# vainglorygame/analyzer

Hardware: AMD Instinct MI355X
Metric: matches/sec rated (whole node), 3v3 TrueSkill, 1M-player roster (higher is better)
Workload: dtype fp32; 1 GPU; global_batch=10000000, seq_len=6, players=1000000, matches_per_gpu=10000000, team_size=3, parallelism=dp1, mode=exact, bench_config=2, skew=1, force_merge=False

## Files before the change

analyzer_amd/csrc/common.h:

```cpp
#pragma once

#include <stdint.h>

#include <type_traits>

#ifndef ANA_DIAG_BUILD
#define ANA_DIAG_BUILD 0
#endif

#if defined(__HIPCC__)
#include <hip/hip_runtime.h>
#define ANA_HD __host__ __device__ __forceinline__
#else
#define ANA_HD inline
#endif

namespace ana {

constexpr int kTracks = 7;
constexpr int kGranules = 8;
constexpr int kRowFloats = 32;
constexpr int kBaseFloats = 16;
constexpr int kLinkWords = 1;
constexpr uint32_t kNoMatch = 0x0fffffffu;
constexpr uint32_t kMatchMask = 0x0fffffffu;
constexpr uint32_t kLinkHasPred = 1u << 30;
constexpr uint32_t kNone = 0xffffffffu;
constexpr int kSlotBits = 28;
constexpr int64_t kMaxSlots = 1ll << kSlotBits;
constexpr int kModes = 6;
constexpr int kModeUnsupported = 255;
constexpr int kVstTiers = 31;
constexpr int kMaxTeamSize = 5;

enum Status : uint8_t {
  kRated = 0,
  kAfk = 1,
  kInvalidRosters = 2,
  kUnsupportedMode = 3,
  kErrSeed = 4,
  kErrSigma = 5,
  kErrEmptyRoster = 6,
  kErrNumeric = 7,
  kErrBadRecord = 8,
  kNotProcessed = 255,
};

struct RateParams {
  float beta2;
  float tau2;
  float unknown_sigma;
  int32_t num_players;
  int64_t num_matches;
  int32_t record_first_prior;
  int32_t epoch;
  const int32_t* epoch_ptr;
  const float* vst;
  int32_t idle_spins;
  int32_t tight_groups;
  int32_t local_handoff;
  int32_t diag;
  uint64_t* progress;
  uint64_t progress_value;
  int64_t progress_at;
  int32_t chunk_len;
  int32_t ctrl_ready;
};

struct RateOut {
  float* quality;
  uint8_t* status;
  float* s_mu;
  float* s_sig;
  float* delta;
  float* m_mu;
  float* m_sig;
  int64_t row;
  int64_t qrow;
  int64_t srow;
};

ANA_HD int meta_mode(uint32_t m0) { return (int)(m0 & 0xffu); }
ANA_HD int meta_n0(uint32_t m0) { return (int)((m0 >> 8) & 0xffu); }
ANA_HD int meta_n1(uint32_t m0) { return (int)((m0 >> 16) & 0xffu); }
ANA_HD int meta_nrosters(uint32_t m0) { return (int)((m0 >> 24) & 0xffu); }
ANA_HD bool meta_winner0(uint32_t m1) { return (m1 & 1u) != 0; }
ANA_HD bool meta_winner1(uint32_t m1) { return (m1 & 2u) != 0; }
ANA_HD bool meta_afk(uint32_t m1) { return (m1 & 4u) != 0; }
ANA_HD uint32_t pack_meta0(int mode, int n0, int n1, int nrosters) {
  return (uint32_t)(mode & 0xff) | ((uint32_t)(n0 & 0xff) << 8) |
         ((uint32_t)(n1 & 0xff) << 16) | ((uint32_t)(nrosters & 0xff) << 24);
}
ANA_HD uint32_t pack_meta1(bool w0, bool w1, uint32_t afk_mask) {
  return (w0 ? 1u : 0u) | (w1 ? 2u : 0u) | (afk_mask ? 4u : 0u) | ((afk_mask & 0xffffffu) << 8);
}

template <int K>
ANA_HD uint8_t early_status(const int32_t* r, int64_t P) {
  constexpr int S = 2 * K;
  const uint32_t m0 = (uint32_t)r[S], m1 = (uint32_t)r[S + 1];
  const int n0 = meta_n0(m0), n1 = meta_n1(m0);
  bool bad = n0 > K || n1 > K;
#pragma unroll
  for (int j = 0; j < S; ++j) {
    const int pos = j < K ? j : j - K;
    if (pos < (j < K ? n0 : n1) && (r[j] < 0 || (int64_t)r[j] >= P)) bad = true;
  }
  if (meta_mode(m0) >= kModes) return kUnsupportedMode;
  if (bad) return kErrBadRecord;
  if (meta_nrosters(m0) != 2) return kInvalidRosters;
  if (meta_afk(m1)) return kAfk;
  return kRated;
}

ANA_HD uint8_t early_status_k(const int32_t* r, int S, int64_t P) {
  switch (S / 2) {
    case 1: return early_status<1>(r, P);
    case 2: return early_status<2>(r, P);
    case 3: return early_status<3>(r, P);
    case 4: return early_status<4>(r, P);
    case 5: return early_status<5>(r, P);
    default: return kErrBadRecord;
  }
}

template <class F>
inline bool with_team_size(int K, F&& f) {
  switch (K) {
    case 1: f(std::integral_constant<int, 1>{}); return true;
    case 2: f(std::integral_constant<int, 2>{}); return true;
    case 3: f(std::integral_constant<int, 3>{}); return true;
    case 4: f(std::integral_constant<int, 4>{}); return true;
    case 5: f(std::integral_constant<int, 5>{}); return true;
    default: return false;
  }
}
static_assert(kMaxTeamSize == 5, "with_team_size and early_status_k list the team sizes");

inline bool window_ok(int K, int64_t W, int64_t M, int64_t P) {
  return K >= 1 && K <= kMaxTeamSize && W >= 5 * 2 * K + 2 && M >= 0 && P >= 0 && P <= 0x7fffffffll;
}
inline bool window_slots_ok(int K, int64_t W, int64_t M, int64_t P) {
  return window_ok(K, W, M, P) && M * 2 * K <= kMaxSlots;
}
inline bool sorted_slots_ok(int K, int64_t n, int64_t P) {
  return K >= 1 && K <= kMaxTeamSize && n >= 0 && n <= kMaxSlots && n % (2 * K) == 0 && P >= 0 && P <= 0x7fffffffll;
}

ANA_HD uint64_t mix64(uint64_t z) {
  z += 0x9e3779b97f4a7c15ull;
  z = (z ^ (z >> 30)) * 0xbf58476d1ce4e5b9ull;
  z = (z ^ (z >> 27)) * 0x94d049bb133111ebull;
  return z ^ (z >> 31);
}
ANA_HD uint64_t rng_u64(uint64_t seed, uint64_t index, uint32_t field) {
  return mix64(mix64(seed ^ (0xd1b54a32d192ed03ull * (uint64_t)(field + 1))) + index);
}
ANA_HD float rng_unit(uint64_t seed, uint64_t index, uint32_t field) {
  return (float)(rng_u64(seed, index, field) >> 40) * (1.0f / 16777216.0f);
}

}
```

analyzer_amd/csrc/radix_sort.hip:

```cpp
#include <hip/hip_runtime.h>

#include <cstdlib>

#include "common.h"
#include "kernels.h"
#include "record_dev.h"

namespace ana {

namespace {

constexpr int kThreads = 512;
constexpr int kWaves = kThreads / 64;
constexpr int kItems = 16;
constexpr int kTile = kThreads * kItems;
constexpr int kRadixBits = 8;
constexpr int kRadix = 1 << kRadixBits;
static_assert(kRadix <= kThreads, "one digit per thread");

__device__ __forceinline__ int64_t xcd_tile(int64_t tiles) {
  const int64_t i = blockIdx.x, q = tiles >> 3, r = tiles & 7, x = i & 7;
  return x * q + (x < r ? x : r) + (i >> 3);
}

template <bool NT>
__device__ __forceinline__ uint32_t ld32(const uint32_t* p) {
  if constexpr (NT) return __builtin_nontemporal_load(p);
  else return *p;
}

__device__ __forceinline__ uint32_t block_exclusive_scan(uint32_t x, uint32_t* wsum,
                                                         uint32_t* total) {
  const int lane = threadIdx.x & 63, wv = threadIdx.x >> 6;
  uint32_t inc = x;
#pragma unroll
  for (int off = 1; off < 64; off <<= 1) {
    const uint32_t y = __shfl_up(inc, off);
    if (lane >= off) inc += y;
  }
  if (lane == 63) wsum[wv] = inc;
  __syncthreads();
  uint32_t before = 0, all = 0;
#pragma unroll
  for (int w = 0; w < kWaves; ++w) {
    if (w < wv) before += wsum[w];
    all += wsum[w];
  }
  if (total) *total = all;
  __syncthreads();
  return before + inc - x;
}

template <int KS>
__device__ __forceinline__ void decode_tile_keys(const int32_t* __restrict__ rec, uint32_t kend,
                                                 int64_t base, int64_t n, uint32_t* lk, uint32_t knone) {
  constexpr int S = 2 * KS, R = S + 2;
  const uint32_t lo = (uint32_t)base;
  const uint32_t hi = (uint32_t)(base + kTile < n ? base + kTile : n);
  const uint32_t m_lo = lo / S, m_hi = (hi + S - 1) / S;
  for (uint32_t m = m_lo + threadIdx.x; m < m_hi; m += kThreads) {
    uint32_t key[S];
    sched_slot_keys<KS>(rec + (int64_t)m * R, (int64_t)kend, knone, key);
#pragma unroll
    for (int j = 0; j < S; ++j) {
      const uint32_t slot = m * S + j;
      if (slot >= lo && slot < hi) lk[slot - lo] = key[j];
    }
  }
}

struct SchedInit {
  int32_t* deps = nullptr;
  uint32_t* ctrl = nullptr;
  int nz = 0;
  int32_t* epoch_bump = nullptr;
};

template <int KS, bool NT = false>
__global__ void __launch_bounds__(kThreads)
radix_upsweep(const uint32_t* __restrict__ keys, const int32_t* __restrict__ rec, uint32_t kend,
              int64_t n, int shift, uint32_t* __restrict__ counts, int64_t tiles, SchedInit init = {},
              uint32_t knone = 0u) {
  __shared__ uint32_t hist[kWaves][kRadix];
  __shared__ uint32_t lkeys[KS > 0 ? kTile : 1];
  const int tid = threadIdx.x, wv = tid >> 6;
  for (int i = tid; i < kWaves * kRadix; i += kThreads) (&hist[0][0])[i] = 0u;
  const int64_t tile = xcd_tile(tiles);
  const int64_t base = tile * kTile;
  if constexpr (KS > 0) {
    if (init.deps) {
      constexpr int S = 2 * KS;
      const int64_t hi = base + kTile < n ? base + kTile : n;
      for (int64_t m = (base + S - 1) / S + tid; m < (hi + S - 1) / S; m += kThreads) init.deps[m] = 0;
    }
    if (blockIdx.x == 0) {
      if (tid < init.nz) init.ctrl[tid] = 0u;
      if (tid == 0 && init.epoch_bump) init.epoch_bump[0] += 1;
    }
  }
  if constexpr (KS > 0) decode_tile_keys<KS>(rec, kend, base, n, lkeys, knone ? knone : kend);
  __syncthreads();
#pragma unroll
  for (int k = 0; k < kItems; ++k) {
    const int64_t idx = base + k * kThreads + tid;
    if (idx < n) {
      const uint32_t key = KS > 0 ? lkeys[k * kThreads + tid] : ld32<NT>(keys + idx);
      atomicAdd(&hist[wv][(key >> shift) & (kRadix - 1)], 1u);
    }
  }
  __syncthreads();
#pragma unroll
  for (int d = tid; d < kRadix; d += kThreads) {
    uint32_t c = 0;
#pragma unroll
    for (int w = 0; w < kWaves; ++w) c += hist[w][d];
    counts[(int64_t)d * tiles + tile] = c;
  }
}

__global__ void __launch_bounds__(kThreads)
radix_rowscan(uint32_t* __restrict__ counts, int64_t tiles, uint32_t* __restrict__ totals) {
  __shared__ uint32_t wsum[kWaves];
  constexpr int kPer = 4;
  uint32_t* row = counts + (int64_t)blockIdx.x * tiles;
  uint32_t carry = 0;
  for (int64_t start = 0; start < tiles; start += kThreads * kPer) {
    uint32_t v[kPer], s = 0;
#pragma unroll
    for (int q = 0; q < kPer; ++q) {
      const int64_t t = start + (int64_t)threadIdx.x * kPer + q;
      v[q] = t < tiles ? row[t] : 0u;
      s += v[q];
    }
    uint32_t all;
    uint32_t ex = carry + block_exclusive_scan(s, wsum, &all);
#pragma unroll
    for (int q = 0; q < kPer; ++q) {
      const int64_t t = start + (int64_t)threadIdx.x * kPer + q;
      if (t < tiles) row[t] = ex;
      ex += v[q];
    }
    carry += all;
  }
  if (threadIdx.x == 0) totals[blockIdx.x] = carry;
}

struct RunEnds {
  uint32_t kf, vf, kl, vl;
};
constexpr uint32_t kRunEmpty = 0xffffffffu;

template <int KS, bool LINK, bool NT = false>
__global__ void __launch_bounds__(kThreads)
radix_downsweep(const uint32_t* __restrict__ kin, const uint32_t* __restrict__ vin,
                const int32_t* __restrict__ rec, uint32_t kend,
                uint32_t* __restrict__ kout, uint32_t* __restrict__ vout, int64_t n, int shift,
                const uint32_t* __restrict__ counts, const uint32_t* __restrict__ totals,
                int64_t tiles, int slots_per_match, uint32_t* __restrict__ link,
                uint32_t vlo = 0u, uint32_t vhi = 0xffffffffu, int bounds = 1,
                RunEnds* __restrict__ bnd = nullptr, int nd = 0, uint32_t knone = 0u) {
  __shared__ uint32_t skey[kTile];
  __shared__ uint32_t sval[kTile];
  __shared__ uint32_t wcnt[kWaves][kRadix];
  __shared__ uint32_t tstart[kRadix];
  __shared__ uint32_t gstart[kRadix];
  __shared__ uint32_t wsum[kWaves];
  const int tid = threadIdx.x, lane = tid & 63, wv = tid >> 6;
  const int64_t tile = xcd_tile(tiles);
  const int64_t base = tile * kTile;
  for (int i = tid; i < kWaves * kRadix; i += kThreads) (&wcnt[0][0])[i] = 0u;
  const bool local_ends = LINK && bnd != nullptr;
  if (!local_ends) {
    const uint32_t below = block_exclusive_scan(tid < kRadix ? totals[tid] : 0u, wsum, nullptr);
    if (tid < kRadix) gstart[tid] = below + counts[(int64_t)tid * tiles + tile];
  }
  if constexpr (KS > 0)
    decode_tile_keys<KS>(rec, kend, base, n, sval, knone ? knone : kend);
  __syncthreads();

  const uint64_t lt_mask = (1ull << lane) - 1ull;
  uint32_t key[kItems], val[kItems], rank[kItems];
#pragma unroll
  for (int it = 0; it < kItems; ++it) {
    const int64_t idx = base + (int64_t)(wv * kItems + it) * 64 + lane;
    const bool valid = idx < n;
    if constexpr (KS > 0) key[it] = valid ? sval[(wv * kItems + it) * 64 + lane] : 0xffffffffu;
    else key[it] = valid ? ld32<NT>(kin + idx) : 0xffffffffu;
    if constexpr (KS == 0) val[it] = valid ? ld32<NT>(vin + idx) : 0u;
    else val[it] = (uint32_t)idx;
  }
#pragma unroll
  for (int it = 0; it < kItems; ++it) {
    const uint32_t d = (key[it] >> shift) & (kRadix - 1);
    uint64_t peers = ~0ull;
#pragma unroll
    for (int b = 0; b < kRadixBits; ++b) {
      const uint64_t bal = __ballot((d >> b) & 1u);
      peers &= ((d >> b) & 1u) ? bal : ~bal;
    }
    const uint32_t before = (uint32_t)__popcll(peers & lt_mask);
    const uint32_t run = wcnt[wv][d];
    rank[it] = run + before;
    if (before == (uint32_t)__popcll(peers) - 1u) wcnt[wv][d] = run + (uint32_t)__popcll(peers);
  }
  __syncthreads();
  {
    uint32_t s = 0;
    if (tid < kRadix) {
#pragma unroll
      for (int w = 0; w < kWaves; ++w) {
        const uint32_t c = wcnt[w][tid];
        wcnt[w][tid] = s;
        s += c;
      }
    }
    const uint32_t ts = block_exclusive_scan(s, wsum, nullptr);
    if (tid < kRadix) tstart[tid] = ts;
  }
  __syncthreads();
#pragma unroll
  for (int it = 0; it < kItems; ++it) {
    const uint32_t d = (key[it] >> shift) & (kRadix - 1);
    const uint32_t pos = tstart[d] + wcnt[wv][d] + rank[it];
    skey[pos] = key[it];
    sval[pos] = val[it];
  }
  __syncthreads();
  const int64_t nvalid = n - base < kTile ? n - base : kTile;
  if constexpr (LINK) {
    if (local_ends && bounds && tid < nd) {
      const uint32_t e = tid + 1 < kRadix ? tstart[tid + 1] : (uint32_t)kTile;
      if (tstart[tid] == e) bnd[tile * nd + tid].kf = kRunEmpty;
    }
  }
#pragma unroll
  for (int k = 0; k < kItems; ++k) {
    const int i = k * kThreads + tid;
    if (i < nvalid) {
      const uint32_t kk = skey[i];
      const uint32_t d = (kk >> shift) & (kRadix - 1);
      const int64_t o = local_ends ? 0 : (int64_t)gstart[d] + (i - (int64_t)tstart[d]);
      if constexpr (!LINK) {
        kout[o] = kk;
        vout[o] = sval[i];
      } else {
        const int hi = d + 1 < (uint32_t)kRadix ? (int)tstart[d + 1] : kTile;
        const bool first = i == (int)tstart[d];
        const bool last = i + 1 == hi || i + 1 >= nvalid;
        const uint32_t v = sval[i];
        if (bounds && (first || last)) {
          if (local_ends) {
            if ((int)d < nd) {
              RunEnds* r = bnd + tile * nd + d;
              if (first) { r->kf = kk; r->vf = v; }
              if (last) { r->kl = kk; r->vl = v; }
            }
          } else {
            kout[o] = kk;
            vout[o] = v;
          }
        }
        if (kk < kend && v >= vlo && v < vhi) {
          uint32_t w = (!last && skey[i + 1] == kk) ? sval[i + 1] / (uint32_t)slots_per_match
                                                     : kNoMatch;
          if (!first && skey[i - 1] == kk) w |= kLinkHasPred;
          link[v] = w;
        }
      }
    }
  }
}

static int link_parts(int64_t n) {
  if (const char* e = getenv("ANA_LINK_PARTS")) {
    const int v = atoi(e);
    if (v >= 1) return v > 16 ? 16 : v;
  }
  const int64_t bytes = n * 4, part = 256ll << 20;
  return (int)((bytes + part - 1) / part);
}

__global__ void __launch_bounds__(kThreads)
sched_fixup(const uint32_t* __restrict__ kout, const uint32_t* __restrict__ vout, int64_t n,
            uint32_t kend, const uint32_t* __restrict__ counts, const uint32_t* __restrict__ totals,
            int64_t tiles, int slots_per_match, uint32_t* __restrict__ link) {
  __shared__ uint32_t wsum[kWaves];
  const int d = blockIdx.y;
  const uint32_t tot = totals[d];
  if (tot == 0) return;
  uint32_t below = 0;
#pragma unroll
  for (int j = threadIdx.x; j < kRadix; j += kThreads) below += j < d ? totals[j] : 0u;
  uint32_t all = 0;
  const uint32_t before = block_exclusive_scan(below, wsum, &all);
  (void)before;
  const uint32_t dstart = all;
  const int64_t t = (int64_t)blockIdx.x * kThreads + threadIdx.x;
  if (t >= tiles) return;
  const uint32_t* row = counts + (int64_t)d * tiles;
  const uint32_t c0 = row[t];
  const uint32_t c1 = t + 1 < tiles ? row[t + 1] : tot;
  if (c1 == c0) return;
  const int64_t of = (int64_t)dstart + c0, ol = (int64_t)dstart + c1 - 1;
  const uint32_t kf = kout[of], kl = kout[ol];
  const bool pred = kf < kend && of > 0 && kout[of - 1] == kf;
  const bool succ = kl < kend && ol + 1 < n && kout[ol + 1] == kl;
  const uint32_t nxt = succ ? vout[ol + 1] / (uint32_t)slots_per_match : kNoMatch;
  if (of == ol) {
    if (kf < kend) link[vout[of]] = nxt | (pred ? kLinkHasPred : 0u);
    return;
  }
  if (pred) {
    const uint32_t v = vout[of];
    link[v] |= kLinkHasPred;
  }
  if (succ) {
    const uint32_t v = vout[ol];
    link[v] = (link[v] & ~kMatchMask) | nxt;
  }
}

constexpr int kRunsMaxDigits = 32;

__global__ void __launch_bounds__(kThreads)
sched_runs_last(const RunEnds* __restrict__ bnd, int64_t tiles, int nd, int32_t* __restrict__ seglast) {
  __shared__ int32_t wmax[kWaves];
  const int d = blockIdx.y;
  const int64_t t = (int64_t)blockIdx.x * kThreads + threadIdx.x;
  int32_t x = (t < tiles && bnd[t * nd + d].kf != kRunEmpty) ? (int32_t)t : -1;
#pragma unroll
  for (int off = 32; off >= 1; off >>= 1) x = max(x, __shfl_xor(x, off));
  if ((threadIdx.x & 63) == 0) wmax[threadIdx.x >> 6] = x;
  __syncthreads();
  if (threadIdx.x == 0) {
    int32_t m = wmax[0];
#pragma unroll
    for (int w = 1; w < kWaves; ++w) m = max(m, wmax[w]);
    seglast[(int64_t)d * gridDim.x + blockIdx.x] = m;
  }
}

__global__ void __launch_bounds__(kThreads)
sched_runs_fixup(const RunEnds* __restrict__ bnd, int64_t tiles, int nd, const int32_t* __restrict__ seglast,
                 uint32_t kend, int slots_per_match, uint32_t* __restrict__ link) {
  __shared__ int32_t wmax[kWaves];
  __shared__ int32_t carry_s;
  const int d = blockIdx.y, lane = threadIdx.x & 63, wv = threadIdx.x >> 6;
  const int64_t seg = blockIdx.x;
  if (wv == 0) {
    int32_t c = -1;
    for (int64_t q = lane; q < seg; q += 64) c = max(c, seglast[(int64_t)d * gridDim.x + q]);
#pragma unroll
    for (int off = 32; off >= 1; off >>= 1) c = max(c, __shfl_xor(c, off));
    if (lane == 0) carry_s = c;
  }
  const int64_t t = seg * kThreads + threadIdx.x;
  RunEnds me = {kRunEmpty, 0u, kRunEmpty, 0u};
  if (t < tiles) me = bnd[t * nd + d];
  const bool full = me.kf != kRunEmpty;
  int32_t x = full ? (int32_t)t : -1;
#pragma unroll
  for (int off = 1; off < 64; off <<= 1) {
    const int32_t y = __shfl_up(x, off);
    if (lane >= off) x = max(x, y);
  }
  if (lane == 63) wmax[wv] = x;
  __syncthreads();
  int32_t before = carry_s;
  for (int w = 0; w < wv; ++w) before = max(before, wmax[w]);
  int32_t ex = __shfl_up(x, 1);
  ex = lane == 0 ? -1 : ex;
  const int32_t pred = max(before, ex);
  if (!full || pred < 0 || me.kf >= kend) return;
  const RunEnds pr = bnd[(int64_t)pred * nd + d];
  if (pr.kl != me.kf) return;
  atomicOr(&link[me.vf], kLinkHasPred);
  atomicAnd(&link[pr.vl], ~kMatchMask | (me.vf / (uint32_t)slots_per_match));
}

constexpr int kChainLowBits = 12;
constexpr int kChainRB = 6;
constexpr uint32_t kChainEmpty = 0xffffffffu;
constexpr bool kChainDefault = true;

template <bool VALS = true>
__device__ __forceinline__ void chain_sort_round(const uint32_t (&key)[kItems], const uint32_t (&val)[kItems],
                                                 int shift, uint32_t* skey, uint32_t* sval,
                                                 uint32_t (*wcnt)[1 << kChainRB], uint32_t* tstart,
                                                 uint32_t* wsum) {
  constexpr int kR = 1 << kChainRB;
  static_assert(kR <= kThreads, "one digit per thread in the scan");
  const int tid = threadIdx.x, lane = tid & 63, wv = tid >> 6;
  const uint64_t lt_mask = (1ull << lane) - 1ull;
  for (int i = tid; i < kWaves * kR; i += kThreads) (&wcnt[0][0])[i] = 0u;
  __syncthreads();
  uint32_t rank[kItems];
#pragma unroll
  for (int it = 0; it < kItems; ++it) {
    const uint32_t d = (key[it] >> shift) & (kR - 1);
    uint64_t peers = ~0ull;
#pragma unroll
    for (int b = 0; b < kChainRB; ++b) {
      const uint64_t bal = __ballot((d >> b) & 1u);
      peers &= ((d >> b) & 1u) ? bal : ~bal;
    }
    const uint32_t before = (uint32_t)__popcll(peers & lt_mask);
    const uint32_t run = wcnt[wv][d];
    rank[it] = run + before;
    if (before == (uint32_t)__popcll(peers) - 1u) wcnt[wv][d] = run + (uint32_t)__popcll(peers);
  }
  __syncthreads();
  {
    uint32_t s = 0;
    if (tid < kR) {
#pragma unroll
      for (int w = 0; w < kWaves; ++w) {
        const uint32_t c = wcnt[w][tid];
        wcnt[w][tid] = s;
        s += c;
      }
    }
    const uint32_t ts = block_exclusive_scan(s, wsum, nullptr);
    if (tid < kR) tstart[tid] = ts;
  }
  __syncthreads();
#pragma unroll
  for (int it = 0; it < kItems; ++it) {
    const uint32_t d = (key[it] >> shift) & (kR - 1);
    const uint32_t pos = tstart[d] + wcnt[wv][d] + rank[it];
    skey[pos] = key[it];
    if constexpr (VALS) sval[pos] = val[it];
  }
  __syncthreads();
}

constexpr uint32_t kLinkDeferred = 0xfffffffeu;
constexpr uint32_t kLinkSkip = 0xffffffffu;

template <int KS, bool NT, bool LINES>
__global__ void __launch_bounds__(kThreads)
sched_chain(uint32_t* kio, const uint32_t* __restrict__ vin,
            const int32_t* __restrict__ rec, uint32_t kend, int64_t n, int low,
            const uint32_t* __restrict__ totals, int slots_per_match, uint32_t* __restrict__ link,
            uint32_t vlo, uint32_t vhi, int64_t matches, SchedInit init) {
  constexpr int kR = 1 << kChainRB;
  static_assert(!LINES || KS == 0, "bucket positions need the partition");
  __shared__ uint32_t skey[kTile];
  __shared__ uint32_t sval[kTile];
  __shared__ uint32_t lbuf[LINES ? kTile : 1];
  __shared__ uint32_t last_seen[1 << kChainLowBits];
  __shared__ uint32_t wcnt[kWaves][kR];
  __shared__ uint32_t tstart[kR];
  __shared__ uint32_t wsum[kWaves];
  const int tid = threadIdx.x, lane = tid & 63, wv = tid >> 6;
  const uint32_t lmask = (1u << low) - 1u;
  for (int e = tid; e <= (int)lmask; e += kThreads) last_seen[e] = kChainEmpty;
  int64_t start = 0, cnt = n;
  if constexpr (KS > 0) {
    if (init.deps)
      for (int64_t m = tid; m < matches; m += kThreads) init.deps[m] = 0;
    if (tid < init.nz) init.ctrl[tid] = 0u;
    if (tid == 0 && init.epoch_bump) init.epoch_bump[0] += 1;
  } else {
    uint32_t below = 0;
    const uint32_t x = tid < (int)blockIdx.x ? totals[tid] : 0u;
    block_exclusive_scan(x, wsum, &below);
    start = below;
    cnt = totals[blockIdx.x];
  }
  const uint32_t kbase = LINES ? (uint32_t)blockIdx.x << low : 0u;
  for (int64_t base = 0; base < cnt; base += kTile) {
    const int64_t nvalid = cnt - base < kTile ? cnt - base : kTile;
    uint32_t key[kItems], val[kItems];
    if constexpr (KS > 0) {
      decode_tile_keys<KS>(rec, kend, base, n, sval, kend);
      __syncthreads();
    }
#pragma unroll
    for (int it = 0; it < kItems; ++it) {
      const int p = (wv * kItems + it) * 64 + lane;
      const bool valid = p < nvalid;
      const int64_t idx = start + base + p;
      if constexpr (KS > 0) {
        key[it] = valid ? sval[p] : 0xffffffffu;
        val[it] = (uint32_t)idx;
      } else if constexpr (!LINES) {
        key[it] = valid ? ld32<NT>(kio + idx) : 0xffffffffu;
        val[it] = valid ? ld32<NT>(vin + idx) : 0u;
      } else {
        key[it] = valid ? (ld32<NT>(kio + idx) & lmask) | (uint32_t)p << low : 0xffffffffu;
        if (valid) sval[p] = ld32<NT>(vin + idx);
      }
    }
    chain_sort_round<!LINES>(key, val, 0, skey, sval, wcnt, tstart, wsum);
    if (low > kChainRB) {
#pragma unroll
      for (int it = 0; it < kItems; ++it) {
        const int p = (wv * kItems + it) * 64 + lane;
        key[it] = skey[p];
        if constexpr (!LINES) val[it] = sval[p];
      }
      chain_sort_round<!LINES>(key, val, kChainRB, skey, sval, wcnt, tstart, wsum);
    }
    uint32_t is_last = 0u, has = 0u;
    if constexpr (!LINES) {
#pragma unroll 2
      for (int k = 0; k < kItems; ++k) {
        const int i = k * kThreads + tid;
        if (i < nvalid) {
          const uint32_t kk = skey[i];
          if (kk < kend) {
            const uint32_t v = sval[i];
            const bool next = i + 1 < nvalid && skey[i + 1] == kk;
            bool pred = i > 0 && skey[i - 1] == kk;
            if (!pred) {
              const uint32_t t = last_seen[kk & lmask];
              if (t != kChainEmpty) {
                pred = true;
                const uint32_t ts = t & kMatchMask;
                if (ts >= vlo && ts < vhi) link[ts] = v / (uint32_t)slots_per_match | (t & kLinkHasPred);
              }
            }
            if (next) {
              if (v >= vlo && v < vhi)
                link[v] = sval[i + 1] / (uint32_t)slots_per_match | (pred ? kLinkHasPred : 0u);
            } else {
              is_last |= 1u << k;
            }
            if (pred) has |= 1u << k;
          }
        }
      }
      __syncthreads();
#pragma unroll 2
      for (int k = 0; k < kItems; ++k) {
        const int i = k * kThreads + tid;
        if (is_last >> k & 1u) last_seen[skey[i] & lmask] = sval[i] | (has >> k & 1u ? kLinkHasPred : 0u);
      }
    } else {
      const int64_t prev = base - kTile;
#pragma unroll 2
      for (int k = 0; k < kItems; ++k) {
        const int i = k * kThreads + tid;
        if (i < nvalid) {
          const uint32_t kl = skey[i] & lmask;
          if ((kbase | kl) < kend) {
            const bool next = i + 1 < nvalid && (skey[i + 1] & lmask) == kl;
            bool pred = i > 0 && (skey[i - 1] & lmask) == kl;
            if (!pred) {
              const uint32_t t = last_seen[kl];
              if (t != kChainEmpty) {
                pred = true;
                const int64_t tp = t & kMatchMask;
                const uint32_t w = sval[skey[i] >> low] / (uint32_t)slots_per_match | (t & kLinkHasPred);
                if (tp >= prev) lbuf[tp - prev] = w;
                else kio[start + tp] = w;
              }
            }
            if (!next) is_last |= 1u << k;
            if (pred) has |= 1u << k;
          }
        }
      }
      __syncthreads();
      if (base > 0) {
#pragma unroll 2
        for (int k = 0; k < kItems; ++k) {
          const int j = k * kThreads + tid;
          const uint32_t w = lbuf[j];
          if (w != kLinkDeferred) *(kio + start + prev + j) = w;
        }
      }
#pragma unroll 2
      for (int k = 0; k < kItems; ++k) {
        const int i = k * kThreads + tid;
        if (is_last >> k & 1u) {
          const uint32_t kk = skey[i];
          last_seen[kk & lmask] = (uint32_t)(base + (kk >> low)) | (has >> k & 1u ? kLinkHasPred : 0u);
        }
      }
      __syncthreads();
#pragma unroll 2
      for (int k = 0; k < kItems; ++k) {
        const int i = k * kThreads + tid;
        if (i < nvalid) {
          const uint32_t kk = skey[i];
          uint32_t w = kLinkSkip;
          if ((kbase | (kk & lmask)) < kend)
            w = is_last >> k & 1u ? kLinkDeferred
                                  : sval[skey[i + 1] >> low] / (uint32_t)slots_per_match |
                                        (has >> k & 1u ? kLinkHasPred : 0u);
          lbuf[kk >> low] = w;
        }
      }
    }
    __syncthreads();
  }
  __syncthreads();
  if constexpr (!LINES) {
    for (int e = tid; e <= (int)lmask; e += kThreads) {
      const uint32_t t = last_seen[e];
      if (t != kChainEmpty) {
        const uint32_t ts = t & kMatchMask;
        if (ts >= vlo && ts < vhi) link[ts] = kNoMatch | (t & kLinkHasPred);
      }
    }
  } else {
    const int64_t lastb = cnt > 0 ? (cnt - 1) / kTile * kTile : 0;
    for (int e = tid; e <= (int)lmask; e += kThreads) {
      const uint32_t t = last_seen[e];
      if (t != kChainEmpty) {
        const int64_t tp = t & kMatchMask;
        const uint32_t w = kNoMatch | (t & kLinkHasPred);
        if (tp >= lastb) lbuf[tp - lastb] = w;
        else kio[start + tp] = w;
      }
    }
    __syncthreads();
    for (int64_t j = tid; j < cnt - lastb; j += kThreads) *(kio + start + lastb + j) = lbuf[j];
  }
}

template <bool NT>
__global__ void __launch_bounds__(kThreads)
sched_unpartition(const uint32_t* __restrict__ lk, const uint32_t* __restrict__ vo, int64_t n,
                  const uint32_t* __restrict__ counts, const uint32_t* __restrict__ totals,
                  int64_t tiles, int nb, uint32_t* __restrict__ link) {
  __shared__ uint32_t out[kTile];
  __shared__ uint32_t tstart[kRadix];
  __shared__ uint32_t gstart[kRadix];
  __shared__ uint32_t wsum[kWaves];
  const int tid = threadIdx.x;
  const int64_t tile = xcd_tile(tiles);
  const int64_t base = tile * kTile;
  const int64_t nvalid = n - base < kTile ? n - base : kTile;
  uint32_t c0 = 0u, len = 0u;
  if (tid < nb) {
    c0 = counts[(int64_t)tid * tiles + tile];
    len = (tile + 1 < tiles ? counts[(int64_t)tid * tiles + tile + 1] : totals[tid]) - c0;
  }
  uint32_t nchain = 0u;
  const uint32_t g = block_exclusive_scan(tid < kRadix ? totals[tid] : 0u, wsum, nullptr);
  const uint32_t ts = block_exclusive_scan(len, wsum, &nchain);
  if (tid < kRadix) {
    gstart[tid] = g + c0;
    tstart[tid] = ts;
  }
#pragma unroll
  for (int k = 0; k < kItems; ++k) out[k * kThreads + tid] = kLinkSkip;
  __syncthreads();
#pragma unroll 4
  for (int k = 0; k < kItems; ++k) {
    const uint32_t i = k * kThreads + tid;
    if (i < nchain) {
      uint32_t d = 0u;
#pragma unroll
      for (uint32_t step = kRadix >> 1; step > 0u; step >>= 1)
        if (tstart[d + step] <= i) d += step;
      const int64_t o = (int64_t)gstart[d] + (i - tstart[d]);
      if (o < n) {
        const uint32_t at = ld32<NT>(vo + o) - (uint32_t)base;
        if (at < (uint32_t)kTile) out[at] = ld32<NT>(lk + o);
      }
    }
  }
  __syncthreads();
#pragma unroll
  for (int k = 0; k < kItems / 4; ++k) {
    const int j = (k * kThreads + tid) * 4;
    const uint4 w = *reinterpret_cast<const uint4*>(out + j);
    const bool all = w.x != kLinkSkip && w.y != kLinkSkip && w.z != kLinkSkip && w.w != kLinkSkip;
    if (j + 4 <= nvalid && all && (reinterpret_cast<uintptr_t>(link + base + j) & 15u) == 0u) {
      *reinterpret_cast<uint4*>(link + base + j) = w;
    } else {
      if (j < nvalid && w.x != kLinkSkip) link[base + j] = w.x;
      if (j + 1 < nvalid && w.y != kLinkSkip) link[base + j + 1] = w.y;
      if (j + 2 < nvalid && w.z != kLinkSkip) link[base + j + 2] = w.z;
      if (j + 3 < nvalid && w.w != kLinkSkip) link[base + j + 3] = w.w;
    }
  }
}

}

size_t radix_sort_workspace_bytes(int64_t n) {
  const int64_t tiles = (n + kTile - 1) / kTile;
  return (size_t)(tiles * kRadix + kRadix) * 4;
}

int launch_radix_sort_pairs(uint32_t* keys, uint32_t* vals, uint32_t* keys_alt, uint32_t* vals_alt,
                            int64_t n, int bits, void* ws, int* result_in_alt, hipStream_t s) {
  *result_in_alt = 0;
  if (n <= 0) return 0;
  if (n > 0x7fffffffLL || bits < 1 || bits > 32) return (int)hipErrorInvalidValue;
  const int64_t tiles = (n + kTile - 1) / kTile;
  uint32_t* counts = static_cast<uint32_t*>(ws);
  uint32_t* totals = counts + tiles * kRadix;
  uint32_t *ki = keys, *vi = vals, *ko = keys_alt, *vo = vals_alt;
  for (int shift = 0; shift < bits; shift += 8) {
    hipLaunchKernelGGL(radix_upsweep<0>, dim3((unsigned)tiles), dim3(kThreads), 0, s, ki, nullptr,
                       0u, n, shift, counts, tiles);
    hipLaunchKernelGGL(radix_rowscan, dim3(kRadix), dim3(kThreads), 0, s, counts, tiles, totals);
    hipLaunchKernelGGL((radix_downsweep<0, false>), dim3((unsigned)tiles), dim3(kThreads), 0, s, ki,
                       vi, nullptr, 0u, ko, vo, n, shift, counts, totals, tiles, 1, nullptr);
    std::swap(ki, ko);
    std::swap(vi, vo);
    *result_in_alt ^= 1;
  }
  return (int)hipGetLastError();
}

template <int K, bool NT>
static void sched_sort_k(const int32_t* rec, int64_t n, uint32_t kend, int bits, uint32_t* ka,
                         uint32_t* va, uint32_t* kb, uint32_t* vb, uint32_t* counts,
                         int64_t tiles, uint32_t* link, const SchedInit& init, bool chain,
                         hipStream_t s) {
  constexpr int S = 2 * K;
  uint32_t* totals = counts + tiles * kRadix;
  const dim3 grid((unsigned)tiles), block(kThreads);
  const uint32_t *ki = nullptr, *vi = nullptr;
  uint32_t *ko = kb, *vo = vb;
  if (chain) {
    const int low = bits < kChainLowBits ? bits : kChainLowBits, top = bits - low;
    if (top > 0) {
      const uint32_t nb = ((kend - 1u) >> low) + 1u;
      const uint32_t knone = nb < (uint32_t)kRadix ? nb << low : kend;
      hipLaunchKernelGGL((radix_upsweep<K, NT>), grid, block, 0, s, nullptr, rec, kend, n, low, counts, tiles,
                         init, knone);
      hipLaunchKernelGGL(radix_rowscan, dim3(kRadix), block, 0, s, counts, tiles, totals);
      hipLaunchKernelGGL((radix_downsweep<K, false, NT>), grid, block, 0, s, nullptr, nullptr, rec, kend, ko,
                         vo, n, low, counts, totals, tiles, S, nullptr, 0u, 0xffffffffu, 1, nullptr, 0, knone);
      if constexpr (NT) {
        hipLaunchKernelGGL((sched_chain<0, NT, true>), dim3(nb), block, 0, s, ko, vo, nullptr, kend, n, low,
                           totals, S, nullptr, 0u, 0xffffffffu, n / S, SchedInit{});
        hipLaunchKernelGGL(sched_unpartition<NT>, grid, block, 0, s, ko, vo, n, counts, totals, tiles,
                           (int)nb, link);
      } else {
        const int parts = link_parts(n);
        for (int q = 0; q < parts; ++q)
          hipLaunchKernelGGL((sched_chain<0, NT, false>), dim3(nb), block, 0, s, ko, vo, nullptr, kend, n, low,
                             totals, S, link, (uint32_t)(n * q / parts), (uint32_t)(n * (q + 1) / parts),
                             n / S, SchedInit{});
      }
    } else {
      const int parts = link_parts(n);
      for (int q = 0; q < parts; ++q)
        hipLaunchKernelGGL((sched_chain<K, NT, false>), dim3(1), block, 0, s, nullptr, nullptr, rec, kend, n, low,
                           nullptr, S, link, (uint32_t)(n * q / parts), (uint32_t)(n * (q + 1) / parts),
                           n / S, q == 0 ? init : SchedInit{});
    }
    return;
  }
  for (int shift = 0; shift < bits; shift += kRadixBits) {
    const bool first = shift == 0, last = shift + kRadixBits >= bits;
    const int nd = bits - shift < kRadixBits ? 1 << (bits - shift) : kRadix;
    if (last && !first && nd <= kRunsMaxDigits) {
      RunEnds* bnd = reinterpret_cast<RunEnds*>(counts);
      const int64_t nseg = (tiles + kThreads - 1) / kThreads;
      int32_t* seglast = reinterpret_cast<int32_t*>(bnd + tiles * nd);
      const int parts = link_parts(n);
      for (int q = 0; q < parts; ++q)
        hipLaunchKernelGGL((radix_downsweep<0, true, NT>), grid, block, 0, s, ki, vi, nullptr, kend, ko, vo,
                           n, shift, counts, totals, tiles, S, link, (uint32_t)(n * q / parts),
                           (uint32_t)(n * (q + 1) / parts), q == 0 ? 1 : 0, bnd, nd);
      const dim3 sgrid((unsigned)nseg, (unsigned)nd);
      hipLaunchKernelGGL(sched_runs_last, sgrid, block, 0, s, bnd, tiles, nd, seglast);
      hipLaunchKernelGGL(sched_runs_fixup, sgrid, block, 0, s, bnd, tiles, nd, seglast, kend, S, link);
      break;
    }
    if (first)
      hipLaunchKernelGGL((radix_upsweep<K, NT>), grid, block, 0, s, nullptr, rec, kend, n, shift, counts, tiles,
                         init);
    else
      hipLaunchKernelGGL((radix_upsweep<0, NT>), grid, block, 0, s, ki, nullptr, kend, n, shift, counts, tiles);
    hipLaunchKernelGGL(radix_rowscan, dim3(kRadix), block, 0, s, counts, tiles, totals);
    const int parts = last ? link_parts(n) : 1;
    if (first && last)
      for (int q = 0; q < parts; ++q)
        hipLaunchKernelGGL((radix_downsweep<K, true, NT>), grid, block, 0, s, nullptr, nullptr, rec, kend, ko,
                           vo, n, shift, counts, totals, tiles, S, link, (uint32_t)(n * q / parts),
                           (uint32_t)(n * (q + 1) / parts), q == 0 ? 1 : 0);
    else if (first)
      hipLaunchKernelGGL((radix_downsweep<K, false, NT>), grid, block, 0, s, nullptr, nullptr, rec, kend, ko,
                         vo, n, shift, counts, totals, tiles, S, nullptr);
    else if (last)
      for (int q = 0; q < parts; ++q)
        hipLaunchKernelGGL((radix_downsweep<0, true, NT>), grid, block, 0, s, ki, vi, nullptr, kend, ko, vo,
                           n, shift, counts, totals, tiles, S, link, (uint32_t)(n * q / parts),
                           (uint32_t)(n * (q + 1) / parts), q == 0 ? 1 : 0);
    else
      hipLaunchKernelGGL((radix_downsweep<0, false, NT>), grid, block, 0, s, ki, vi, nullptr, kend, ko, vo, n,
                         shift, counts, totals, tiles, S, nullptr);
    if (last)
      hipLaunchKernelGGL(sched_fixup, dim3((unsigned)((tiles + kThreads - 1) / kThreads), kRadix), block,
                         0, s, ko, vo, n, kend, counts, totals, tiles, S, link);
    ki = ko;
    vi = vo;
    ko = ko == kb ? ka : kb;
    vo = vo == vb ? va : vb;
  }
}

int launch_sched_sort(int K, const int32_t* rec, int64_t M, uint32_t num_players, uint32_t* ka,
                      uint32_t* va, uint32_t* kb, uint32_t* vb, void* ws, uint32_t* link,
                      hipStream_t s, int32_t* deps, uint32_t* ctrl, int nz, int32_t* epoch_bump,
                      int sort_nt) {
  const int64_t n = M * 2 * K;
  if (n <= 0) return 0;
  if (n > kMaxSlots) return (int)hipErrorInvalidValue;
  int bits = 1;
  while (bits < 32 && (1ull << bits) <= (uint64_t)num_players) ++bits;
  const int64_t tiles = (n + kTile - 1) / kTile;
  uint32_t* counts = static_cast<uint32_t*>(ws);
  SchedInit init;
  init.deps = deps;
  init.ctrl = ctrl;
  init.nz = ctrl ? nz : 0;
  init.epoch_bump = epoch_bump;
  const char* nt_e = getenv("ANA_SORT_NT");
  const int nt = nt_e ? atoi(nt_e) : sort_nt >= 0 ? sort_nt : 0;
  if (nt != 0 && nt != 2) return (int)hipErrorInvalidValue;
  const char* chain_e = getenv("ANA_SCHED_CHAIN");
  const int top = bits > kChainLowBits ? bits - kChainLowBits : 0;
  const bool chain_pays = (n >> top) <= 2 * kTile + n / 128;
  const bool chain = (chain_e ? atoi(chain_e) != 0 : kChainDefault && chain_pays) && bits <= 20;
  const bool known = with_team_size(K, [&](auto k) {
    constexpr int kK = decltype(k)::value;
    if (nt == 2) sched_sort_k<kK, true>(rec, n, num_players, bits, ka, va, kb, vb, counts, tiles, link, init, chain, s);
    else sched_sort_k<kK, false>(rec, n, num_players, bits, ka, va, kb, vb, counts, tiles, link, init, chain, s);
  });
  return known ? (int)hipGetLastError() : (int)hipErrorInvalidValue;
}

}
```

Measured before the change: 1.757 billion matches/s.

## Restructure chain scheduler: one-pass class sort, wave-per-class ballot linking, magic division

Replaces the two-round 6-bit LDS sort in sched_chain with a single 3-bit class sort where each wave owns one key class. Predecessor and successor detection now uses ballot matching on the remaining key bits within each wave instead of neighbour comparisons over sorted shared memory. The link buffer becomes a double-size ring so deferred links write in place, removing several barrier-separated passes. Integer division by slots per match is replaced with a precomputed magic multiply. This aims to cut LDS traffic, barriers and divides, at the cost of a larger shared footprint and more complex correctness conditions, for example load imbalance across the class waves.

Result: no change. 1.766 billion matches/s (median of 6 runs) (+0.5%).

```diff
diff --git a/analyzer_amd/csrc/common.h b/analyzer_amd/csrc/common.h
--- a/analyzer_amd/csrc/common.h
+++ b/analyzer_amd/csrc/common.h
@@ -28,6 +28,10 @@
 constexpr uint32_t kNone = 0xffffffffu;
 constexpr int kSlotBits = 28;
 constexpr int64_t kMaxSlots = 1ll << kSlotBits;
+ANA_HD uint32_t slot_div_magic(uint32_t slots_per_match) {
+  return (uint32_t)((0x100000000ull + slots_per_match - 1u) / slots_per_match);
+}
+ANA_HD uint32_t slot_div(uint32_t v, uint32_t magic) { return (uint32_t)(((uint64_t)v * magic) >> 32); }
 constexpr int kModes = 6;
 constexpr int kModeUnsupported = 255;
 constexpr int kVstTiers = 31;
diff --git a/analyzer_amd/csrc/radix_sort.hip b/analyzer_amd/csrc/radix_sort.hip
--- a/analyzer_amd/csrc/radix_sort.hip
+++ b/analyzer_amd/csrc/radix_sort.hip
@@ -379,59 +379,64 @@
 }
 
 constexpr int kChainLowBits = 12;
-constexpr int kChainRB = 6;
+constexpr int kChainClassBits = 3;
+static_assert(1 << kChainClassBits == kWaves, "one wave per player class");
 constexpr uint32_t kChainEmpty = 0xffffffffu;
 constexpr bool kChainDefault = true;
 
-template <bool VALS = true>
-__device__ __forceinline__ void chain_sort_round(const uint32_t (&key)[kItems], const uint32_t (&val)[kItems],
-                                                 int shift, uint32_t* skey, uint32_t* sval,
-                                                 uint32_t (*wcnt)[1 << kChainRB], uint32_t* tstart,
-                                                 uint32_t* wsum) {
-  constexpr int kR = 1 << kChainRB;
-  static_assert(kR <= kThreads, "one digit per thread in the scan");
+__device__ __forceinline__ void match_bit(uint32_t x, int b, uint32_t& plo, uint32_t& phi) {
+  const uint32_t m = (uint32_t)((int32_t)(x << (31 - b)) >> 31);
+  const uint64_t bal = __ballot(m != 0u);
+  plo &= ~((uint32_t)bal ^ m);
+  phi &= ~((uint32_t)(bal >> 32) ^ m);
+}
+
+template <int RB>
+__device__ __forceinline__ void chain_sort_round(const uint32_t (&key)[kItems], uint32_t dmask, uint32_t* skey,
+                                                 uint32_t* wcnt, uint32_t* tstart) {
+  constexpr int kR = 1 << RB;
+  static_assert(kWaves * kR == 64, "the scan below: one lane of wave 0 per (wave, digit)");
   const int tid = threadIdx.x, lane = tid & 63, wv = tid >> 6;
-  const uint64_t lt_mask = (1ull << lane) - 1ull;
-  for (int i = tid; i < kWaves * kR; i += kThreads) (&wcnt[0][0])[i] = 0u;
-  __syncthreads();
   uint32_t rank[kItems];
 #pragma unroll
   for (int it = 0; it < kItems; ++it) {
-    const uint32_t d = (key[it] >> shift) & (kR - 1);
-    uint64_t peers = ~0ull;
-#pragma unroll
-    for (int b = 0; b < kChainRB; ++b) {
-      const uint64_t bal = __ballot((d >> b) & 1u);
-      peers &= ((d >> b) & 1u) ? bal : ~bal;
-    }
-    const uint32_t before = (uint32_t)__popcll(peers & lt_mask);
-    const uint32_t run = wcnt[wv][d];
+    const uint32_t d = key[it] & dmask;
+    uint32_t plo = ~0u, phi = ~0u;
+#pragma unroll
+    for (int b = 0; b < RB; ++b) match_bit(d, b, plo, phi);
+    const uint32_t before = __builtin_amdgcn_mbcnt_hi(phi, __builtin_amdgcn_mbcnt_lo(plo, 0u));
+    uint32_t* c = wcnt + (wv << RB) + d;
+    const uint32_t run = *c;
     rank[it] = run + before;
-    if (before == (uint32_t)__popcll(peers) - 1u) wcnt[wv][d] = run + (uint32_t)__popcll(peers);
-  }
-  __syncthreads();
-  {
-    uint32_t s = 0;
-    if (tid < kR) {
-#pragma unroll
-      for (int w = 0; w < kWaves; ++w) {
-        const uint32_t c = wcnt[w][tid];
-        wcnt[w][tid] = s;
-        s += c;
-      }
-    }
-    const uint32_t ts = block_exclusive_scan(s, wsum, nullptr);
-    if (tid < kR) tstart[tid] = ts;
-  }
-  __syncthreads();
-#pragma unroll
-  for (int it = 0; it < kItems; ++it) {
-    const uint32_t d = (key[it] >> shift) & (kR - 1);
-    const uint32_t pos = tstart[d] + wcnt[wv][d] + rank[it];
-    skey[pos] = key[it];
-    if constexpr (VALS) sval[pos] = val[it];
-  }
-  __syncthreads();
+    *c = run + (uint32_t)__popc(plo) + (uint32_t)__popc(phi);
+  }
+  __syncthreads();
+  if (wv == 0) {
+    const int d = lane & (kR - 1);
+    const uint32_t c = wcnt[lane];
+    uint32_t inc = c;
+#pragma unroll
+    for (int off = kR; off < 64; off <<= 1) {
+      const uint32_t y = __shfl_up(inc, off);
+      if (lane >= off) inc += y;
+    }
+    const uint32_t tot = __shfl(inc, 64 - kR + d);
+    uint32_t sc = tot;
+#pragma unroll
+    for (int off = 1; off < kR; off <<= 1) {
+      const uint32_t y = __shfl_up(sc, off);
+      if (lane >= off) sc += y;
+    }
+    const uint32_t ts = __shfl(sc - tot, d);
+    wcnt[lane] = ts + inc - c;
+    if (lane < kR) tstart[lane] = ts;
+    if (lane == 0) tstart[kR] = (uint32_t)kTile;
+  }
+  __syncthreads();
+#pragma unroll
+  for (int it = 0; it < kItems; ++it) skey[wcnt[(wv << RB) + (key[it] & dmask)] + rank[it]] = key[it];
+  __syncthreads();
+  if (tid < 64) wcnt[tid] = 0u;
 }
 
 constexpr uint32_t kLinkDeferred = 0xfffffffeu;
@@ -441,20 +446,24 @@
 __global__ void __launch_bounds__(kThreads)
 sched_chain(uint32_t* kio, const uint32_t* __restrict__ vin,
             const int32_t* __restrict__ rec, uint32_t kend, int64_t n, int low,
-            const uint32_t* __restrict__ totals, int slots_per_match, uint32_t* __restrict__ link,
+            const uint32_t* __restrict__ totals, uint32_t div_magic, uint32_t* __restrict__ link,
             uint32_t vlo, uint32_t vhi, int64_t matches, SchedInit init) {
-  constexpr int kR = 1 << kChainRB;
+  constexpr int kR = 1 << kChainClassBits;
+  constexpr uint32_t kRing = 2 * kTile - 1;
   static_assert(!LINES || KS == 0, "bucket positions need the partition");
   __shared__ uint32_t skey[kTile];
   __shared__ uint32_t sval[kTile];
-  __shared__ uint32_t lbuf[LINES ? kTile : 1];
+  __shared__ uint32_t lbuf[LINES ? 2 * kTile : 1];
   __shared__ uint32_t last_seen[1 << kChainLowBits];
-  __shared__ uint32_t wcnt[kWaves][kR];
-  __shared__ uint32_t tstart[kR];
+  __shared__ uint32_t wcnt[kWaves * kR];
+  __shared__ uint32_t tstart[kR + 1];
   __shared__ uint32_t wsum[kWaves];
   const int tid = threadIdx.x, lane = tid & 63, wv = tid >> 6;
   const uint32_t lmask = (1u << low) - 1u;
+  const uint32_t dmask = lmask < (uint32_t)(kR - 1) ? lmask : (uint32_t)(kR - 1);
+  const uint64_t gt_mask = ~0ull << lane << 1;
   for (int e = tid; e <= (int)lmask; e += kThreads) last_seen[e] = kChainEmpty;
+  if (tid < kWaves * kR) wcnt[tid] = 0u;
   int64_t start = 0, cnt = n;
   if constexpr (KS > 0) {
     if (init.deps)
@@ -468,129 +477,111 @@
     start = below;
     cnt = totals[blockIdx.x];
   }
-  const uint32_t kbase = LINES ? (uint32_t)blockIdx.x << low : 0u;
+  const uint32_t kbase = KS > 0 ? 0u : (uint32_t)blockIdx.x << low;
+  __syncthreads();
   for (int64_t base = 0; base < cnt; base += kTile) {
     const int64_t nvalid = cnt - base < kTile ? cnt - base : kTile;
-    uint32_t key[kItems], val[kItems];
+    uint32_t key[kItems];
     if constexpr (KS > 0) {
       decode_tile_keys<KS>(rec, kend, base, n, sval, kend);
       __syncthreads();
     }
-#pragma unroll
-    for (int it = 0; it < kItems; ++it) {
-      const int p = (wv * kItems + it) * 64 + lane;
-      const bool valid = p < nvalid;
-      const int64_t idx = start + base + p;
-      if constexpr (KS > 0) {
-        key[it] = valid ? sval[p] : 0xffffffffu;
-        val[it] = (uint32_t)idx;
-      } else if constexpr (!LINES) {
-        key[it] = valid ? ld32<NT>(kio + idx) : 0xffffffffu;
-        val[it] = valid ? ld32<NT>(vin + idx) : 0u;
-      } else {
-        key[it] = valid ? (ld32<NT>(kio + idx) & lmask) | (uint32_t)p << low : 0xffffffffu;
-        if (valid) sval[p] = ld32<NT>(vin + idx);
-      }
-    }
-    chain_sort_round<!LINES>(key, val, 0, skey, sval, wcnt, tstart, wsum);
-    if (low > kChainRB) {
+    if (KS == 0 && nvalid == kTile) {
 #pragma unroll
       for (int it = 0; it < kItems; ++it) {
         const int p = (wv * kItems + it) * 64 + lane;
-        key[it] = skey[p];
-        if constexpr (!LINES) val[it] = sval[p];
-      }
-      chain_sort_round<!LINES>(key, val, kChainRB, skey, sval, wcnt, tstart, wsum);
-    }
-    uint32_t is_last = 0u, has = 0u;
-    if constexpr (!LINES) {
-#pragma unroll 2
-      for (int k = 0; k < kItems; ++k) {
-        const int i = k * kThreads + tid;
-        if (i < nvalid) {
-          const uint32_t kk = skey[i];
-          if (kk < kend) {
-            const uint32_t v = sval[i];
-            const bool next = i + 1 < nvalid && skey[i + 1] == kk;
-            bool pred = i > 0 && skey[i - 1] == kk;
+        key[it] = (ld32<NT>(kio + start + base + p) & lmask) | (uint32_t)p << low;
+        sval[p] = ld32<NT>(vin + start + base + p);
+      }
+    } else {
+#pragma unroll
+      for (int it = 0; it < kItems; ++it) {
+        const uint32_t p = (wv * kItems + it) * 64 + lane;
+        const bool valid = p < (uint32_t)nvalid;
+        if constexpr (KS > 0) {
+          key[it] = valid ? (sval[p] & lmask) | p << low : 0xffffffffu;
+        } else {
+          key[it] = valid ? (ld32<NT>(kio + start + base + p) & lmask) | p << low : 0xffffffffu;
+          if (valid) sval[p] = ld32<NT>(vin + start + base + p);
+        }
+      }
+    }
+    chain_sort_round<kChainClassBits>(key, dmask, skey, wcnt, tstart);
+    {
+      const int64_t prev = base - kTile;
+      const uint32_t s0 = __builtin_amdgcn_readfirstlane(tstart[wv]);
+      uint32_t s1 = __builtin_amdgcn_readfirstlane(tstart[wv + 1]);
+      s1 = s1 < (uint32_t)nvalid ? s1 : (uint32_t)nvalid;
+      const auto key_at = [&](uint32_t i) { return skey[i < (uint32_t)kTile ? i : (uint32_t)kTile - 1u]; };
+      const auto slot_of = [&](uint32_t k) { return KS > 0 ? (uint32_t)base + (k >> low) : sval[k >> low & (kTile - 1)]; };
+      uint32_t kk = key_at(s0 + lane), kk_n = key_at(s0 + 64u + lane);
+      uint32_t v = slot_of(kk);
+      for (uint32_t b = s0; b < s1; b += 64) {
+        const uint32_t kk_nn = key_at(b + 128u + lane), v_n = slot_of(kk_n);
+        const bool valid = b + lane < s1;
+        const uint32_t p = kk >> low, kl = kk & lmask;
+        const bool live = valid && (kbase | kl) < kend;
+        const uint32_t mm = slot_div(v, div_magic);
+        const uint64_t lb = __ballot(live);
+        uint32_t plo = (uint32_t)lb, phi = (uint32_t)(lb >> 32);
+#pragma unroll
+        for (int bit = kChainClassBits; bit < kChainLowBits; ++bit) match_bit(kl, bit, plo, phi);
+        bool pred = __builtin_amdgcn_mbcnt_hi(phi, __builtin_amdgcn_mbcnt_lo(plo, 0u)) != 0u;
+        const uint64_t above = ((uint64_t)phi << 32 | plo) & gt_mask;
+        const uint32_t sm = __shfl(mm, above ? __builtin_ctzll(above) : lane);
+        if constexpr (!LINES) {
+          if (live) {
             if (!pred) {
-              const uint32_t t = last_seen[kk & lmask];
+              const uint32_t t = last_seen[kl];
               if (t != kChainEmpty) {
                 pred = true;
                 const uint32_t ts = t & kMatchMask;
-                if (ts >= vlo && ts < vhi) link[ts] = v / (uint32_t)slots_per_match | (t & kLinkHasPred);
+                if (ts >= vlo && ts < vhi) link[ts] = mm | (t & kLinkHasPred);
               }
             }
-            if (next) {
-              if (v >= vlo && v < vhi)
-                link[v] = sval[i + 1] / (uint32_t)slots_per_match | (pred ? kLinkHasPred : 0u);
+            if (above) {
+              if (v >= vlo && v < vhi) link[v] = sm | (pred ? kLinkHasPred : 0u);
             } else {
-              is_last |= 1u << k;
+              last_seen[kl] = v | (pred ? kLinkHasPred : 0u);
             }
-            if (pred) has |= 1u << k;
           }
-        }
-      }
-      __syncthreads();
-#pragma unroll 2
-      for (int k = 0; k < kItems; ++k) {
-        const int i = k * kThreads + tid;
-        if (is_last >> k & 1u) last_seen[skey[i] & lmask] = sval[i] | (has >> k & 1u ? kLinkHasPred : 0u);
-      }
-    } else {
-      const int64_t prev = base - kTile;
-#pragma unroll 2
-      for (int k = 0; k < kItems; ++k) {
-        const int i = k * kThreads + tid;
-        if (i < nvalid) {
-          const uint32_t kl = skey[i] & lmask;
-          if ((kbase | kl) < kend) {
-            const bool next = i + 1 < nvalid && (skey[i + 1] & lmask) == kl;
-            bool pred = i > 0 && (skey[i - 1] & lmask) == kl;
+        } else {
+          const uint32_t at = ((uint32_t)base + p) & kRing;
+          if (live) {
             if (!pred) {
               const uint32_t t = last_seen[kl];
               if (t != kChainEmpty) {
                 pred = true;
                 const int64_t tp = t & kMatchMask;
-                const uint32_t w = sval[skey[i] >> low] / (uint32_t)slots_per_match | (t & kLinkHasPred);
-                if (tp >= prev) lbuf[tp - prev] = w;
+                const uint32_t w = mm | (t & kLinkHasPred);
+                if (tp >= prev) lbuf[(uint32_t)tp & kRing] = w;
                 else kio[start + tp] = w;
               }
             }
-            if (!next) is_last |= 1u << k;
-            if (pred) has |= 1u << k;
+            if (above) {
+              lbuf[at] = sm | (pred ? kLinkHasPred : 0u);
+            } else {
+              lbuf[at] = kLinkDeferred;
+              last_seen[kl] = (uint32_t)(base + p) | (pred ? kLinkHasPred : 0u);
+            }
+          } else if (valid) {
+            lbuf[at] = kLinkSkip;
           }
         }
-      }
-      __syncthreads();
-      if (base > 0) {
-#pragma unroll 2
-        for (int k = 0; k < kItems; ++k) {
-          const int j = k * kThreads + tid;
-          const uint32_t w = lbuf[j];
-          if (w != kLinkDeferred) *(kio + start + prev + j) = w;
-        }
-      }
-#pragma unroll 2
-      for (int k = 0; k < kItems; ++k) {
-        const int i = k * kThreads + tid;
-        if (is_last >> k & 1u) {
-          const uint32_t kk = skey[i];
-          last_seen[kk & lmask] = (uint32_t)(base + (kk >> low)) | (has >> k & 1u ? kLinkHasPred : 0u);
-        }
-      }
-      __syncthreads();
-#pragma unroll 2
-      for (int k = 0; k < kItems; ++k) {
-        const int i = k * kThreads + tid;
-        if (i < nvalid) {
-          const uint32_t kk = skey[i];
-          uint32_t w = kLinkSkip;
-          if ((kbase | (kk & lmask)) < kend)
-            w = is_last >> k & 1u ? kLinkDeferred
-                                  : sval[skey[i + 1] >> low] / (uint32_t)slots_per_match |
-                                        (has >> k & 1u ? kLinkHasPred : 0u);
-          lbuf[kk >> low] = w;
+        kk = kk_n;
+        kk_n = kk_nn;
+        v = v_n;
+      }
+      if constexpr (LINES) {
+        __syncthreads();
+        if (base > 0) {
+          const uint32_t* pl = lbuf + ((uint32_t)prev & kRing);
+#pragma unroll 4
+          for (int k = 0; k < kItems; ++k) {
+            const int j = k * kThreads + tid;
+            const uint32_t w = pl[j];
+            if (w != kLinkDeferred) *(kio + start + prev + j) = w;
+          }
         }
       }
     }
@@ -612,12 +603,13 @@
       if (t != kChainEmpty) {
         const int64_t tp = t & kMatchMask;
         const uint32_t w = kNoMatch | (t & kLinkHasPred);
-        if (tp >= lastb) lbuf[tp - lastb] = w;
+        if (tp >= lastb) lbuf[(uint32_t)tp & kRing] = w;
         else kio[start + tp] = w;
       }
     }
     __syncthreads();
-    for (int64_t j = tid; j < cnt - lastb; j += kThreads) *(kio + start + lastb + j) = lbuf[j];
+    const uint32_t* pl = lbuf + ((uint32_t)lastb & kRing);
+    for (int64_t j = tid; j < cnt - lastb; j += kThreads) *(kio + start + lastb + j) = pl[j];
   }
 }
 
@@ -732,21 +724,21 @@
                          vo, n, low, counts, totals, tiles, S, nullptr, 0u, 0xffffffffu, 1, nullptr, 0, knone);
       if constexpr (NT) {
         hipLaunchKernelGGL((sched_chain<0, NT, true>), dim3(nb), block, 0, s, ko, vo, nullptr, kend, n, low,
-                           totals, S, nullptr, 0u, 0xffffffffu, n / S, SchedInit{});
+                           totals, slot_div_magic(S), nullptr, 0u, 0xffffffffu, n / S, SchedInit{});
         hipLaunchKernelGGL(sched_unpartition<NT>, grid, block, 0, s, ko, vo, n, counts, totals, tiles,
                            (int)nb, link);
       } else {
         const int parts = link_parts(n);
         for (int q = 0; q < parts; ++q)
           hipLaunchKernelGGL((sched_chain<0, NT, false>), dim3(nb), block, 0, s, ko, vo, nullptr, kend, n, low,
-                             totals, S, link, (uint32_t)(n * q / parts), (uint32_t)(n * (q + 1) / parts),
+                             totals, slot_div_magic(S), link, (uint32_t)(n * q / parts), (uint32_t)(n * (q + 1) / parts),
                              n / S, SchedInit{});
       }
     } else {
       const int parts = link_parts(n);
       for (int q = 0; q < parts; ++q)
         hipLaunchKernelGGL((sched_chain<K, NT, false>), dim3(1), block, 0, s, nullptr, nullptr, rec, kend, n, low,
-                           nullptr, S, link, (uint32_t)(n * q / parts), (uint32_t)(n * (q + 1) / parts),
+                           nullptr, slot_div_magic(S), link, (uint32_t)(n * q / parts), (uint32_t)(n * (q + 1) / parts),
                            n / S, q == 0 ? init : SchedInit{});
     }
     return;
```
